# PeterFWS/Structure-PLP-SLAM

Measured on AMD Instinct MI355X. Metric: frames/sec ORB+LSD extract+match, 640x480 TUM-RGBD, 1/2/4/8 GPU, higher is better.
Workload: dtype u8

## Files before the change

structure-plp-slam_amd/csrc/line_context.hip:

```cpp
#include <hip/hip_runtime.h>

#include <algorithm>
#include <cmath>
#include <cstring>
#include <mutex>
#include <vector>

#include "line_device.hpp"
#include "null4.hpp"
#include "seed_sort_model.hpp"
#include "sincos_ziv.hpp"
#include "plp_common.hpp"

using namespace plp;

struct plp_line {
    HostPinned pin;
    int device = 0;
    hipStream_t stream = nullptr;
    hipStream_t idle_stream = nullptr;
    int rows = 0, cols = 0, capB = 0;
    int grow_waves = 0;
    int seed_order = PLP_SEED_ORDER_LIBSTDCXX;
    bool mw_ok = false, seed_sort_ok = false;
// ... 3 lines not shown
    ResizeExactTab rt{};
    BlurTapsN t11{}, t5{};
    LbdWeightsDev w{};
    DevBuf tabs, blur11, scaled, pix, g2, maxgrad, undef, order, n_order, reg, mw_heap, seed_ent, seed_ws, raw, n_raw, dx, dy, all_kl, all_kl_dir, all_lbd, n_all, status, prof, grow_stats;
    DevBuf l0copy, s_kl, s_lbd, s_fn, s_cnt;
    DevBuf aligned;
    int s_cap = 0;
    int last_B = 0;
    bool last_profiled = false;
    hipStream_t last_stream = nullptr;
    bool profiling = false;
    bool grow_big_ok = false;
    hipEvent_t ev[9] = {};
    double stage_ms[9] = {0, 0, 0, 0, 0, 0, 0, 0, 0};
    long stage_batches = 0;
    std::mutex mu;
};

namespace {

void gaussian_taps(int n, double sigma, int* out) {
    std::vector<double> k(n);
    double sum = 0;
    for (int i = 0; i < n; ++i) { const double x = i - (n - 1) * 0.5; k[i] = std::exp(-0.5 / (sigma * sigma) * x * x); sum += k[i]; }
    double err = 0;
    int acc = 0;
    for (int i = 0; i < n / 2; ++i) {
        const double adj = k[i] / sum * 256.0 + err;
        const int v = (int)std::nearbyint(adj);
        err = adj - v;
        out[i] = out[n - 1 - i] = v;
        acc += v;
    }
    out[n / 2] = 256 - 2 * acc;
}

int floor_d(double v) { int i = (int)v; return i - (i > v); }

void exact_coeffs(int ssize, int dsize, std::vector<int16_t>& ofs, std::vector<int16_t>& c1) {
    const double scale = 1.0 / ((double)dsize / ssize);
    for (int d = 0; d < dsize; ++d) {
        const double val = ((double)d + 0.5) * scale - 0.5;
        const int iv = floor_d(val);
        if (iv >= 0 && ssize > 1) {
            if (iv < ssize - 1) { ofs.push_back((int16_t)iv); c1.push_back((int16_t)std::nearbyint((val - (double)iv) * 256.0)); }
            else { ofs.push_back((int16_t)(ssize - 1)); c1.push_back(-1); }
        } else { ofs.push_back(0); c1.push_back(-2); }
    }
}

plp_status build(plp_line* c, int rows, int cols) {
    if (c->rows == rows && c->cols == cols) return PLP_OK;
    if (rows < 16 || cols < 16 || rows > 16000 || cols > 16000) return set_error(PLP_ERR_INVALID_ARG, "unsupported frame size for the line front-end");
    LinePlanes& P = c->P;
    P.W = cols; P.H = rows;
    P.sw = (int)std::nearbyint(cols * 0.5); P.sh = (int)std::nearbyint(rows * 0.5);
    P.sw_magic = (P.sw >= 2 && P.sw <= 8192) ? (uint32_t)(((1ull << 32) + (uint64_t)P.sw - 1) / (uint64_t)P.sw) : 0u;
    if (P.sw >= 65536 || P.sh >= 65536 || (size_t)P.sw * P.sh > kLsdMaxScaledPixels || (!c->grow_big_ok && (size_t)P.sw * P.sh > 516065))
        return set_error(PLP_ERR_UNSUPPORTED, "frame too large for the LSD region-growing kernel (the half-resolution image must not exceed 524,257 pixels: a 1920 x 1080 frame is the largest common one)");
    P.pitch = (cols + 63) / 64 * 64; P.spitch = (P.sw + 63) / 64 * 64;
    LsdParams& lp = c->lp;
    const double ang_th = 22.5, quant = 2.0;
    lp.prec = M_PI * ang_th / 180; lp.p = ang_th / 180; lp.rho = quant / std::sin(lp.prec);
    lp.c_pass = (float)std::cos(lp.prec - kLsdAngleBand); lp.c_fail = (float)std::cos(lp.prec + kLsdAngleBand);
    {
        uint32_t g = 0;
        while (g < 600000u && std::sqrt((double)g / 4.0) <= lp.rho) ++g;
        lp.g2_def_min = g;
    }
    lp.density_th = 0.6; lp.scale = 0.5; lp.n_bins = 1024; lp.refine = 1;
    const double LOG_NT = 5 * (std::log10((double)P.sw) + std::log10((double)P.sh)) / 2 + std::log10(11.0);
    lp.min_reg_size = (int)(size_t)(-LOG_NT / std::log10(lp.p));
    lp.min_length = (float)(0.125 * std::min(cols, rows));
    lp.keep_length = 60.f;
    const double sigma = 0.6 / 0.5;
    const unsigned h = (unsigned)std::ceil(sigma * std::sqrt(2 * 3.0 * std::log(10.0)));
    if (h != 5) return set_error(PLP_ERR_UNSUPPORTED, "unexpected LSD kernel size");
    gaussian_taps(11, sigma, c->t11.k);
    for (int i = 0; i < 11; ++i) c->t5.k[i] = 0;
    gaussian_taps(5, 1.0, c->t5.k);
    {
        double u = (7 * 3 - 1) / 2, sg = (7 * 2 + 1) / 2, inv = -1 / (2 * sg * sg);
        for (int i = 0; i < 21; ++i) { const double d = i - u; c->w.l[i] = (float)std::exp(d * d * inv); }
        u = (9 * 7 - 1) / 2; sg = u; inv = -1 / (2 * sg * sg);
        for (int i = 0; i < 63; ++i) { const double d = i - u; c->w.g[i] = (float)std::exp(d * d * inv); }
    }
    std::vector<int16_t> xo, xc, yo, yc;
    exact_coeffs(cols, P.sw, xo, xc);
    exact_coeffs(rows, P.sh, yo, yc);
    {
        bool plain = cols == 2 * P.sw && rows == 2 * P.sh;
        for (int i = 0; plain && i < P.sw; ++i) plain = xo[i] == 2 * i && xc[i] == 128;
        for (int i = 0; plain && i < P.sh; ++i) plain = yo[i] == 2 * i && yc[i] == 128;
        P.half_exact = plain ? 1 : 0;
    }
    std::vector<int16_t> blob;
    blob.insert(blob.end(), xo.begin(), xo.end()); blob.insert(blob.end(), xc.begin(), xc.end());
    blob.insert(blob.end(), yo.begin(), yo.end()); blob.insert(blob.end(), yc.begin(), yc.end());
    PLP_HIP(c->tabs.upload(blob.data(), blob.size() * 2, c->stream));
    PLP_HIP(hipStreamSynchronize(c->stream));
    const int16_t* base = (const int16_t*)c->tabs.p;
    c->rt.xo = base; c->rt.xc = base + P.sw; c->rt.yo = base + 2 * P.sw; c->rt.yc = base + 2 * P.sw + P.sh;
    c->rows = rows; c->cols = cols; c->capB = 0; c->mw_capB = 0; c->seed_capB = 0;
    return PLP_OK;
}

plp_status ensure(plp_line* c, int B) {
    LinePlanes& P = c->P;
    const size_t n = (size_t)P.sw * P.sh, nv = (size_t)(P.sw - 1) * (P.sh - 1);
    const int Bmw = std::min(B, kLsdMwMaxFrames);
    if (B > c->capB) {
        if (!P.half_exact) PLP_HIP(c->blur11.reserve((size_t)P.pitch * P.H * B));
        PLP_HIP(c->scaled.reserve((size_t)P.spitch * P.sh * B));
        PLP_HIP(c->pix.reserve(n * sizeof(LsdPix) * B));
        PLP_HIP(c->g2.reserve(n * 4 * B)); PLP_HIP(c->n_order.reserve(4 * (size_t)B)); PLP_HIP(c->maxgrad.reserve(4 * ((n + 255) / 256) * (size_t)B)); PLP_HIP(c->undef.reserve((n + 63) / 64 * 8 * B));
        PLP_HIP(c->order.reserve(nv * 4 * B)); PLP_HIP(c->reg.reserve(std::max(n * (size_t)B, 2 * n * (size_t)Bmw) * 4));
        PLP_HIP(c->raw.reserve(sizeof(float4) * kLineCap * B)); PLP_HIP(c->n_raw.reserve(4 * (size_t)B));
        PLP_HIP(c->dx.reserve(dxy_frame_entries(P.W, P.H) * 4 * B));
        PLP_HIP(c->all_kl.reserve(sizeof(plp_keyline) * kLineCap * B)); PLP_HIP(c->all_kl_dir.reserve(sizeof(float2) * kLineCap * B)); PLP_HIP(c->all_lbd.reserve((size_t)32 * kLineCap * B));
        PLP_HIP(c->n_all.reserve(4 * (size_t)B)); PLP_HIP(c->status.reserve(16)); PLP_HIP(c->prof.reserve(128)); PLP_HIP(c->grow_stats.reserve(16 * (size_t)B));
        P.blur11 = (uint8_t*)c->blur11.p; P.scaled = (uint8_t*)c->scaled.p;
        P.pix = (LsdPix*)c->pix.p; P.g2 = (uint32_t*)c->g2.p; P.n_order = (int32_t*)c->n_order.p;
        P.blockmax = (uint32_t*)c->maxgrad.p; P.undef = (unsigned long long*)c->undef.p;
        P.order = (uint32_t*)c->order.p; P.reg = (uint32_t*)c->reg.p; P.raw = (float4*)c->raw.p; P.n_raw = (int32_t*)c->n_raw.p;
        P.dxy = (short2*)c->dx.p; P.all_kl = (plp_keyline*)c->all_kl.p; P.all_kl_dir = (float2*)c->all_kl_dir.p; P.all_lbd = (uint8_t*)c->all_lbd.p;
        P.n_all = (int32_t*)c->n_all.p; P.status = (int32_t*)c->status.p; P.prof = (long long*)c->prof.p; P.grow_stats = (int32_t*)c->grow_stats.p;
        c->capB = B;
    }
    P.reg_frame_stride = B <= kLsdMwMaxFrames ? 2 * n : n;
    P.mw_heap_frame_stride = (size_t)(kMwMaxWaves - 1) * kMwHeapBufs * kMwHeap;
    if (c->mw_ok && B <= kLsdMwMaxFrames && B > c->mw_capB) {
        PLP_HIP(c->mw_heap.reserve(P.mw_heap_frame_stride * 4 * (size_t)B));
        c->mw_capB = B;
    }
    P.mw_heap = (B <= c->mw_capB) ? (uint32_t*)c->mw_heap.p : nullptr;
    if (c->seed_order == PLP_SEED_ORDER_LIBSTDCXX && B > c->seed_capB) {
        PLP_HIP(c->seed_ent.reserve(nv * 4 * (size_t)B)); PLP_HIP(c->seed_ws.reserve(seed_sort_ws_entries(nv) * 4 * (size_t)B));
        c->seed_capB = B;
    }
    return PLP_OK;
}

plp_status run(plp_line* c, const uint8_t* d_imgs, int B, int rows, int cols, size_t step, size_t frame_stride, plp_keyline* d_kl,
               uint8_t* d_lbd, double* d_fn, int cap, int32_t* d_counts, hipStream_t st) {
    PLP_HIP(hipSetDevice(c->device));
    if (c->seed_order == PLP_SEED_ORDER_LIBSTDCXX && !c->seed_sort_ok)
        return set_error(PLP_ERR_UNSUPPORTED, "this device refused the dynamic LDS size of the exact seed sort (144 KB per workgroup): select PLP_SEED_ORDER_STABLE with plp_line_set_seed_order");
    PLP_TRY(build(c, rows, cols));
    PLP_TRY(ensure(c, B));
    if (((uintptr_t)d_imgs % 4 == 0) && (step % 4 == 0) && (frame_stride % 4 == 0)) {
        c->P.img = d_imgs; c->P.img_frame_stride = frame_stride; c->P.img_pitch = (int)step;
    } else {
        const size_t fs = (size_t)c->P.pitch * rows;
        PLP_HIP(c->aligned.reserve(fs * B));
        for (int f = 0; f < B; ++f)
            PLP_HIP(hipMemcpy2DAsync((uint8_t*)c->aligned.p + f * fs, c->P.pitch, d_imgs + f * frame_stride, step, cols, rows, hipMemcpyDeviceToDevice, st));
        c->P.img = (const uint8_t*)c->aligned.p; c->P.img_frame_stride = fs; c->P.img_pitch = c->P.pitch;
    }
    PLP_HIP(hipMemsetAsync(c->status.p, 0, 16, st));
    if (c->profiling) PLP_HIP(hipMemsetAsync(c->prof.p, 0, 128, st));
    const bool exact = c->seed_order == PLP_SEED_ORDER_LIBSTDCXX;
    c->lp.seed_exact = exact ? 1 : 0;
    const SeedSortBufs ssb{(uint32_t*)c->seed_ent.p, (uint32_t*)c->seed_ws.p, seed_sort_ws_entries((size_t)(c->P.sw - 1) * (c->P.sh - 1))};
    launch_line_front(st, c->P, c->lp, c->rt, c->t11, c->t5, c->w, d_kl, d_lbd, d_fn, cap, d_counts, B, c->profiling ? c->ev : nullptr,
                      c->grow_waves, exact ? &ssb : nullptr, c->mw_ok);
    PLP_HIP(hipGetLastError());
    if (c->profiling) {
        PLP_HIP(hipEventSynchronize(c->ev[8]));
        for (int i = 0; i < 8; ++i) { float ms = 0; PLP_HIP(hipEventElapsedTime(&ms, c->ev[i], c->ev[i + 1])); c->stage_ms[i] += ms; }
        float tot = 0; PLP_HIP(hipEventElapsedTime(&tot, c->ev[0], c->ev[8])); c->stage_ms[8] += tot;
        ++c->stage_batches;
    }
    c->last_B = B; c->last_stream = st; c->last_profiled = c->profiling;
    return PLP_OK;
}

plp_status batch_status(const int32_t s[4], bool check_cap) {
    if (check_cap && (s[0] & 1)) return set_error(PLP_ERR_CAPACITY, "a frame produced more lines than `cap`; output truncated");
    if (s[0] & 4) return set_error(PLP_ERR_OVERFLOW, "more LSD segments than the per-frame capacity");
    if (s[0] & 16) return set_error(PLP_ERR_HIP, "region growing with several waves per frame timed out in a wait (protocol error, please report the frame)");
    if (s[0] & 32) {
        static thread_local char msg[320];
        snprintf(msg, sizeof msg, "the exact seed sort stopped short in frame %d of the batch (reason %d: 1 = a partition's swap count / cut failed its check [m = %d], 2-3, 6-8 = a list or stack of its LDS ran out of space, "
                 "4-5 = a wave waited beyond the limit): the seed order of this batch is not guaranteed; please report the frame", s[2], s[1], s[3]);
        return set_error(PLP_ERR_OVERFLOW, msg);
    }
    return PLP_OK;
}

}

extern "C" {

plp_status plp_line_create(int device, plp_line** out) {
    if (!out) return set_error(PLP_ERR_INVALID_ARG, "out is NULL");
    *out = nullptr;
    int n = 0;
    if (hipGetDeviceCount(&n) != hipSuccess || n == 0) return set_error(PLP_ERR_NO_DEVICE, "no HIP device visible: the line front-end has no CPU fallback");
    if (device < 0 || device >= n) return set_error(PLP_ERR_INVALID_ARG, "device index out of range");
    PLP_HIP(hipSetDevice(device));
    plp_line* c = new plp_line();
    c->device = device;
    c->mw_ok = grow_mw_configure() == hipSuccess;
    c->grow_big_ok = grow_configure() == hipSuccess;
    c->seed_sort_ok = seed_sort_configure() == hipSuccess;
    (void)hipGetLastError();
    if (hipStreamCreateWithFlags(&c->stream, hipStreamNonBlocking) != hipSuccess) { delete c; return set_error(PLP_ERR_HIP, "hipStreamCreate failed"); }
    if (hipStreamCreateWithFlags(&c->idle_stream, hipStreamNonBlocking) != hipSuccess) c->idle_stream = nullptr;
    *out = c;
// ... 255 lines not shown
```

structure-plp-slam_amd/csrc/line_device.hpp:

```cpp
#pragma once
#include <hip/hip_runtime.h>
#include <stdint.h>

#include "../../include/plp_front.h"

namespace plp {

constexpr int kMwHeap = 16384;
constexpr int kMwHeapBufs = 2;
constexpr int kMwMaxWaves = 8;
constexpr int kLsdMwMaxFrames = 256;
constexpr int kLineCap = 2048;
constexpr double kLsdNotDef = -1024.0;
constexpr int kLsdSeedPixBits = 20;
constexpr uint32_t kLsdSeedPixMask = (1u << kLsdSeedPixBits) - 1u;
constexpr size_t kLsdGrowLdsBytes = 66560;
constexpr size_t kLsdMaxScaledPixels = (kLsdGrowLdsBytes / 4 - 256) * 32 - 31;
static_assert(kLsdMaxScaledPixels <= (size_t)kLsdSeedPixMask + 1, "seed packing of k_lsd_order must hold every admitted pixel index");
static_assert(kLsdSeedPixBits + 10 <= 32, "10 bits of gradient bin above the pixel field");

struct alignas(16) LsdPix { float deg; uint32_t g2; float2 cs; };
__device__ __forceinline__ double pix_ang(const LsdPix& p) { return (double)p.deg * (3.14159265358979323846 / 180); }
__device__ __forceinline__ double pix_mod(const LsdPix& p) { return sqrt((double)p.g2 / 4.0); }

struct LinePlanes {
    int W, H;
    int sw, sh;
    uint32_t sw_magic;
    int pitch, spitch;
    const uint8_t* img; size_t img_frame_stride; int img_pitch;
    uint8_t* blur11;
    uint8_t* scaled;
    LsdPix* pix;
    uint32_t* g2;
    uint32_t* blockmax;
    unsigned long long* undef;
    uint32_t* order;
    int32_t* n_order;
    uint32_t* reg; size_t reg_frame_stride;
    uint32_t* mw_heap; size_t mw_heap_frame_stride;
    float4* raw; int32_t* n_raw;
    short2* dxy;
    plp_keyline* all_kl; uint8_t* all_lbd; int32_t* n_all;
    float2* all_kl_dir;
    int32_t* status;
    int half_exact;
    int32_t* grow_stats;
    long long* prof;
};

__host__ __device__ inline size_t dxy_frame_entries(int W, int H) { return (size_t)((W + 7) / 8) * ((H + 3) / 4) * 32; }
__host__ __device__ inline int dxy_index(int x, int y, int tiles_x) { return (((y >> 2) * tiles_x + (x >> 3)) << 5) + ((y & 3) << 3) + (x & 7); }

struct LsdParams {
    double prec, p, rho, density_th, scale;
    int n_bins, refine, min_reg_size;
    float min_length;
    float keep_length;
    float c_pass, c_fail;
    uint32_t g2_def_min;
    int seed_exact;
};
constexpr double kLsdAngleBand = 3.5e-4;
constexpr double kLsdBandMinPrec = 0.01, kLsdBandMaxPrec = 1.5;

struct ResizeExactTab { const int16_t *xo, *xc, *yo, *yc; };
struct BlurTapsN { int k[11]; };
struct LbdWeightsDev { float g[63], l[21]; };

struct SeedSortBufs { uint32_t* ent; uint32_t* ws; size_t ws_stride; };
size_t seed_sort_ws_entries(size_t nv);
hipError_t seed_sort_configure();
void launch_seed_order_exact(hipStream_t st, const LinePlanes& P, const LsdParams& lp, int B, uint32_t* ent, uint32_t* ws, size_t ws_stride);
void launch_seed_sort_debug(hipStream_t st, uint32_t* ent, int n, int depth, uint32_t skip_key, uint32_t* ws, int32_t* status, int* dbg, int variant, int copies = 1);
hipError_t grow_mw_configure();
hipError_t grow_configure();

void launch_line_front(hipStream_t st, const LinePlanes& P, const LsdParams& lp, const ResizeExactTab& rt, const BlurTapsN& t11,
                       const BlurTapsN& t5, const LbdWeightsDev& w, plp_keyline* out_kl, uint8_t* out_lbd, double* out_fn, int cap,
                       int32_t* out_counts, int B, hipEvent_t* ev, int grow_waves, const SeedSortBufs* seed_exact, bool mw_ok);

}
```

structure-plp-slam_amd/csrc/line_kernels.hip:

```cpp
#include <hip/hip_runtime.h>
#include <stdint.h>

#include <algorithm>
#include <cstdlib>

#include "blur_tile.hpp"
#include "plp_barrier.hpp"
#include "line_device.hpp"
#include "plp_common.hpp"
#include "sincos_ziv.hpp"
#include "xcd_map.hpp"

namespace plp {

struct TileDiv { uint32_t gx_magic, tiles_x_magic; };
static inline TileDiv tile_div(int tiles, int tiles_x, int B) { return TileDiv{plp_div_magic((uint32_t)tiles, (uint64_t)tiles * B), plp_div_magic((uint32_t)tiles_x, (uint64_t)tiles)}; }

__device__ __forceinline__ int reflect101_l(int p, int len) {
    if (len == 1) return 0;
    while (p < 0 || p >= len) p = p < 0 ? -p : 2 * (len - 1) - p;
    return p;
}

__device__ __forceinline__ float fast_atan2_deg_l(float y, float x) {
// ... 1288 lines not shown
                    e->pos = t; e->n1 = r.n1; e->n2 = r.n2; e->nfinal = r.nfinal; e->flags = (r.keep ? 1u : 0u) | (r.second ? 2u : 0u); e->off = (uint32_t)hoff;
                    e->na = r.na; e->line = r.line;
                }
                if (tot <= kMwInline) {
                    if (lane < acc_n) e->inl[lane] = heap_ld(g.reg + lane);
                    else if (lane < tot) e->inl[lane] = g.assumed[lane - acc_n];
                }
                __builtin_amdgcn_fence(__ATOMIC_RELEASE, PLP_MW_SCOPE_NAME);
                __builtin_amdgcn_wave_barrier();
                ++nent; hoff += (tot + 1) & ~1;
                if (lds_ld(&pend_hi[h]) < 0) lds_st(&pend_lo[h], g.my_pos);
                lds_st(&pend_hi[h], g.my_pos);
                lds_st(&buf_n[h * kMwBufs + kbuf], nent);
                mw_forget(g, g.reg, acc_n, 0);
            } else mw_forget(g, g.reg, acc_n, wv);
            __builtin_amdgcn_wave_barrier();
            {
                const int p = (int)mine;
                const int ow = tent_owner(g, p), owh = ow > kMwPending ? ow - kMwPending : ow;
                const bool skip = committed(p) || (ow != 0 && (ow == kMwMainId || owh == wv || cur_pos[min(owh, kMwMaxWaves) - 1] < grp * kMwGroup + lane));
                todo &= __ballot(!skip);
            }
            lds_st(&hstate[h], (grp << 8) | (t + 1));
        }
    }
    if (is_main) {
        if (lane == 0) {
            P.n_raw[b] = min(n_lines, kLineCap);
            int32_t* gs = P.grow_stats + (size_t)b * 4; gs[0] = n_self; gs[1] = n_spec_ok; gs[2] = n_spec_bad; gs[3] = W;
            if (P.prof && b == 0 && prof_on) {
                P.prof[0] = now() - c_begin; P.prof[1] = c_wait; P.prof[2] = c_self;
                P.prof[3] = (long long)hcount[0] | ((long long)hcount[1] << 32); P.prof[4] = n_self; P.prof[5] = (long long)n_spec_ok | ((long long)n_spec_bad << 32);
                P.prof[6] = c_commit; P.prof[7] = c_pub; P.prof[8] = c_grp; P.prof[9] = P.prof[10] = P.prof[11] = 0;
            }
        }
        lds_st(done, 1);
    }
}

__global__ __launch_bounds__(64) void k_keylines(LinePlanes P, LsdParams lp) {
    const int b = blockIdx.x, lane = threadIdx.x;
    const int n = P.n_raw[b];
    const float4* raw = P.raw + (size_t)b * kLineCap;
    plp_keyline* out = P.all_kl + (size_t)b * kLineCap;
    int run = 0;
    for (int base = 0; base < n; base += 64) {
        const int i = base + lane;
        bool keep = false;
        plp_keyline kl{};
        if (i < n) {
            float4 e = raw[i];
            const float fw = (float)P.W, fh = (float)P.H;
            if (e.x < 0) e.x = 0;
            if (e.x >= fw) e.x = fw - 1.0f;
            if (e.z < 0) e.z = 0;
            if (e.z >= fw) e.z = fw - 1.0f;
            if (e.y < 0) e.y = 0;
            if (e.y >= fh) e.y = fh - 1.0f;
            if (e.w < 0) e.w = 0;
            if (e.w >= fh) e.w = fh - 1.0f;
            const double ddx = (double)__fsub_rn(e.x, e.z), ddy = (double)__fsub_rn(e.y, e.w);
            const double length = (double)(float)sqrt(ddx * ddx + ddy * ddy);
            keep = length > (double)lp.min_length;
            kl.startPointX = e.x; kl.startPointY = e.y; kl.endPointX = e.z; kl.endPointY = e.w;
            kl.sPointInOctaveX = e.x; kl.sPointInOctaveY = e.y; kl.ePointInOctaveX = e.z; kl.ePointInOctaveY = e.w;
            kl.lineLength = (float)length;
            const int x1 = __float2int_rn(e.x), y1 = __float2int_rn(e.y), x2 = __float2int_rn(e.z), y2 = __float2int_rn(e.w);
            kl.numOfPixels = max(abs(x2 - x1), abs(y2 - y1)) + 1;
            kl.angle = (float)atan2((double)__fsub_rn(e.w, e.y), (double)__fsub_rn(e.z, e.x));
            kl.octave = 0;
            kl.size = __fmul_rn(__fsub_rn(e.z, e.x), __fsub_rn(e.w, e.y));
            kl.response = __fdiv_rn(kl.lineLength, (float)max(P.W, P.H));
            kl.pt_x = __fdiv_rn(__fadd_rn(e.z, e.x), 2.0f);
            kl.pt_y = __fdiv_rn(__fadd_rn(e.w, e.y), 2.0f);
        }
        const unsigned long long bal = __ballot(keep);
        if (keep) {
            kl.class_id = run + __popcll(bal & ((1ull << lane) - 1ull));
            out[kl.class_id] = kl;
            P.all_kl_dir[(size_t)b * kLineCap + kl.class_id] = make_float2((float)cos((double)kl.angle), (float)sin((double)kl.angle));
        }
        run += __popcll(bal);
    }
    if (lane == 0) P.n_all[b] = run;
}

constexpr int kSobelTW = 120, kSobelTH = 30;
static_assert(sizeof(BlurTileLds<2>::in) >= kBlurTH * (kBlurTW / 4) * 4, "the blurred tile must fit the input rows it replaces");
__global__ __launch_bounds__(256) __attribute__((amdgpu_waves_per_eu(8, 8))) void k_blur_sobel(const uint8_t* __restrict__ src, size_t src_fs, int src_pitch,
                                                                                            short2* __restrict__ dxy, int w, int h, BlurTapsN taps, TileDiv td) {
    __shared__ __attribute__((aligned(16))) BlurTileLds<2> Sb;
    uint32_t* const bt = reinterpret_cast<uint32_t*>(Sb.in);
    const int tiles_x = (w + kSobelTW - 1) / kSobelTW;
    unsigned t, f;
    xcd_frame_major(t, f, td.gx_magic);
    const int trow = (int)plp_div(t, (unsigned)tiles_x, td.tiles_x_magic);
    const int bx0 = ((int)t - trow * tiles_x) * kSobelTW - 4, by0 = trow * kSobelTH - 1;
    blur_tile_core<2>(Sb, src + (size_t)f * src_fs, src_pitch, w, h, bx0, by0, taps.k, [&](int r0, int c4, const uint32_t (&rows)[kBlurRS]) {
#pragma unroll
        for (int rr = 0; rr < kBlurRS; ++rr) bt[(r0 + rr) * (kBlurTW / 4) + c4 / 4] = rows[rr];
    });
    wg_barrier();
    short2* out_frame = dxy + (size_t)f * dxy_frame_entries(w, h);
    const int tiles8 = (w + 7) / 8;
    for (int i = threadIdx.x; i < (kSobelTW / 4) * (kSobelTH / 2); i += 256) {
        const int cgp = i % (kSobelTW / 4), rp = i / (kSobelTW / 4);
        const int x = bx0 + 4 + 4 * cgp, y = by0 + 1 + 2 * rp;
        if (x >= w || y >= h) continue;
        const int cd = 1 + cgp;
        int d[4][4], sm[4][4];
#pragma unroll
        for (int r = 0; r < 4; ++r) {
            const uint32_t* q = &bt[(2 * rp + r) * (kBlurTW / 4) + cd];
            const uint32_t A = q[-1], Bv = q[0], Cv = q[1];
            const int p[6] = {(int)(A >> 24), (int)(Bv & 255u), (int)((Bv >> 8) & 255u), (int)((Bv >> 16) & 255u), (int)(Bv >> 24), (int)(Cv & 255u)};
#pragma unroll
            for (int k = 0; k < 4; ++k) { d[r][k] = p[k + 2] - p[k]; sm[r][k] = p[k] + 2 * p[k + 1] + p[k + 2]; }
        }
#pragma unroll
        for (int j = 0; j < 2; ++j) {
            if (y + j >= h) continue;
            uint32_t out[4];
#pragma unroll
            for (int k = 0; k < 4; ++k)
                out[k] = ((uint32_t)(d[j][k] + 2 * d[j + 1][k] + d[j + 2][k]) & 0xffffu) | ((uint32_t)(sm[j + 2][k] - sm[j][k]) << 16);
            *reinterpret_cast<uint4*>(out_frame + dxy_index(x, y + j, tiles8)) = make_uint4(out[0], out[1], out[2], out[3]);
        }
    }
}

__constant__ int c_comb[32][2] = {{0, 1}, {0, 2}, {0, 3}, {0, 4}, {0, 5}, {0, 6}, {1, 2}, {1, 3}, {1, 4}, {1, 5}, {1, 6},
                                  {2, 3}, {2, 4}, {2, 5}, {2, 6}, {2, 7}, {2, 8}, {3, 4}, {3, 5}, {3, 6}, {3, 7}, {3, 8},
                                  {4, 5}, {4, 6}, {4, 7}, {4, 8}, {5, 6}, {5, 7}, {5, 8}, {6, 7}, {6, 8}, {7, 8}};

constexpr int kLbdU = 8;
__global__ __launch_bounds__(256) void k_lbd(LinePlanes P, LbdWeightsDev W) {
    __shared__ float s_row[4][63][8];
    __shared__ float s_des[4][72], s_des2[4][72], s_norm[4][4];
    const int lane = threadIdx.x & 63, wv = __builtin_amdgcn_readfirstlane((int)(threadIdx.x >> 6)), b = blockIdx.y;
    const int n_lines = P.n_all[b];
    for (int li = blockIdx.x * 4 + wv; li < n_lines; li += gridDim.x * 4) {
    const plp_keyline kl = P.all_kl[(size_t)b * kLineCap + li];
    const short2* dxyImg = P.dxy + (size_t)b * dxy_frame_entries(P.W, P.H);
    const int tiles8 = (P.W + 7) / 8;
    const short imageWidth = (short)(P.W - 1), imageHeight = (short)(P.H - 1);
    const short lengthOfLSP = (short)kl.numOfPixels;
    const short halfWidth = (short)((lengthOfLSP - 1) / 2), halfHeight = 31;
    const float midX = (float)(0.5 * (double)__fadd_rn(kl.sPointInOctaveX, kl.ePointInOctaveX));
    const float midY = (float)(0.5 * (double)__fadd_rn(kl.sPointInOctaveY, kl.ePointInOctaveY));
    const float2 dir = P.all_kl_dir[(size_t)b * kLineCap + li];
    const float dL0 = dir.x, dL1 = dir.y;
    const float dO0 = -dL1, dO1 = dL0;
    if (lane < 63) {
        float sCorX0 = __fadd_rn(__fadd_rn(__fmul_rn(-dL0, (float)halfWidth), __fmul_rn(dL1, (float)halfHeight)), midX);
        float sCorY0 = __fadd_rn(__fsub_rn(__fmul_rn(-dL1, (float)halfWidth), __fmul_rn(dL0, (float)halfHeight)), midY);
        for (int r = 0; r < lane; ++r) { sCorX0 = __fsub_rn(sCorX0, dL1); sCorY0 = __fadd_rn(sCorY0, dL0); }
        float sCorX = sCorX0, sCorY = sCorY0;
        float pgdL = 0, ngdL = 0, pgdO = 0, ngdO = 0;
        for (int w0 = 0; w0 < lengthOfLSP; w0 += kLbdU) {
            int off[kLbdU];
#pragma unroll
            for (int u = 0; u < kLbdU; ++u) {
                short t = (short)roundf(sCorX);
                const short xCor = (t < 0) ? 0 : (t > imageWidth) ? imageWidth : t;
                t = (short)roundf(sCorY);
                const short yCor = (t < 0) ? 0 : (t > imageHeight) ? imageHeight : t;
                off[u] = dxy_index(xCor, yCor, tiles8);
                sCorX = __fadd_rn(sCorX, dL0);
                sCorY = __fadd_rn(sCorY, dL1);
            }
            short2 vxy[kLbdU];
#pragma unroll
            for (int u = 0; u < kLbdU; ++u) vxy[u] = dxyImg[off[u]];
#pragma unroll
            for (int u = 0; u < kLbdU; ++u) {
                if (w0 + u < lengthOfLSP) {
                    const float fx = (float)vxy[u].x, fy = (float)vxy[u].y;
                    const float gDL = __fadd_rn(__fmul_rn(fx, dL0), __fmul_rn(fy, dL1));
                    const float gDO = __fadd_rn(__fmul_rn(fx, dO0), __fmul_rn(fy, dO1));
                    if (gDL > 0) pgdL = __fadd_rn(pgdL, gDL); else ngdL = __fsub_rn(ngdL, gDL);
                    if (gDO > 0) pgdO = __fadd_rn(pgdO, gDO); else ngdO = __fsub_rn(ngdO, gDO);
                }
            }
        }
        const float cg = W.g[lane];
        pgdL = __fmul_rn(cg, pgdL); ngdL = __fmul_rn(cg, ngdL); pgdO = __fmul_rn(cg, pgdO); ngdO = __fmul_rn(cg, ngdO);
        float* r = s_row[wv][lane];
        r[0] = pgdL; r[1] = ngdL; r[2] = __fmul_rn(pgdL, pgdL); r[3] = __fmul_rn(ngdL, ngdL);
        r[4] = pgdO; r[5] = ngdO; r[6] = __fmul_rn(pgdO, pgdO); r[7] = __fmul_rn(ngdO, ngdO);
    }
    __builtin_amdgcn_fence(__ATOMIC_RELEASE, "workgroup");
    __builtin_amdgcn_wave_barrier();
    for (int item = lane; item < 72; item += 64) {
        const int band = item >> 3, comp = item & 7;
        const bool sq = (comp == 2 || comp == 3 || comp == 6 || comp == 7);
        float acc = 0;
        for (int hID = max(0, (band - 1) * 7); hID < min(63, (band + 2) * 7); ++hID) {
            const int rb = hID / 7;
            const float c = rb == band ? W.l[hID % 7 + 7] : (rb == band + 1 ? W.l[hID % 7 + 14] : W.l[hID % 7]);
            const float v = s_row[wv][hID][comp];
            acc = sq ? __fadd_rn(acc, __fmul_rn(__fmul_rn(c, c), v)) : __fadd_rn(acc, __fmul_rn(c, v));
        }
        s_des[wv][item] = acc;
    }
    __builtin_amdgcn_fence(__ATOMIC_RELEASE, "workgroup");
    __builtin_amdgcn_wave_barrier();
    float* des = s_des2[wv];
    auto wave_sync = [] { __builtin_amdgcn_fence(__ATOMIC_ACQ_REL, "workgroup"); __builtin_amdgcn_wave_barrier(); };
    if (lane < 36) {
        const int band = lane >> 2, k = lane & 3;
        const float invN = (band == 0 || band == 8) ? (float)(1.0 / (7 * 2.0)) : (float)(1.0 / (7 * 3.0));
        const float* sb = &s_des[wv][band * 8];
        const int mi = (k < 2) ? k : k + 2, qi = mi + 2;
        const float temp = __fmul_rn(sb[mi], invN);
        des[band * 8 + k] = temp;
        des[band * 8 + 4 + k] = sqrtf(__fsub_rn(__fmul_rn(sb[qi], invN), __fmul_rn(temp, temp)));
    }
    wave_sync();
    if (lane == 0) {
        float tempM = 0, tempS = 0;
        for (int band = 0; band < 9; ++band) {
            const float* v = des + 8 * band;
            for (int k = 0; k < 4; ++k) tempM = __fadd_rn(tempM, __fmul_rn(v[k], v[k]));
            for (int k = 4; k < 8; ++k) tempS = __fadd_rn(tempS, __fmul_rn(v[k], v[k]));
        }
        s_norm[wv][0] = __fdiv_rn(1.0f, sqrtf(tempM));
        s_norm[wv][1] = __fdiv_rn(1.0f, sqrtf(tempS));
    }
    wave_sync();
    for (int i = lane; i < 72; i += 64) {
        float v = __fmul_rn(des[i], s_norm[wv][(i >> 2) & 1]);
        if ((double)v > 0.4) v = (float)0.4;
        des[i] = v;
    }
    wave_sync();
    if (lane == 0) {
        float temp = 0;
        for (int i = 0; i < 72; ++i) temp = __fadd_rn(temp, __fmul_rn(des[i], des[i]));
        s_norm[wv][2] = __fdiv_rn(1.0f, sqrtf(temp));
    }
    wave_sync();
    for (int i = lane; i < 72; i += 64) des[i] = __fmul_rn(des[i], s_norm[wv][2]);
    wave_sync();
    if (lane < 32) {
        const float* f1 = des + 8 * c_comb[lane][0];
        const float* f2 = des + 8 * c_comb[lane][1];
        unsigned r = 0;
        for (int i = 0; i < 8; ++i) r += (f1[i] > f2[i]) ? (1u << i) : 0u;
        P.all_lbd[((size_t)b * kLineCap + li) * 32 + lane] = (uint8_t)r;
    }
    __builtin_amdgcn_fence(__ATOMIC_ACQ_REL, "workgroup");
    __builtin_amdgcn_wave_barrier();
    }
}

__global__ __launch_bounds__(64) void k_line_finalize(LinePlanes P, LsdParams lp, plp_keyline* __restrict__ out_kl,
                                                      uint8_t* __restrict__ out_lbd, double* __restrict__ out_fn, int cap,
                                                      int32_t* __restrict__ out_counts) {
    const int b = blockIdx.x, lane = threadIdx.x;
    const int n = P.n_all[b];
    int run = 0;
    for (int base = 0; base < n; base += 64) {
        const int i = base + lane;
        plp_keyline kl{};
        bool keep = false;
        if (i < n) { kl = P.all_kl[(size_t)b * kLineCap + i]; keep = kl.octave == 0 && kl.lineLength >= lp.keep_length; }
        const unsigned long long bal = __ballot(keep);
        const int o = run + __popcll(bal & ((1ull << lane) - 1ull));
        if (keep && o < cap) {
            out_kl[(size_t)b * cap + o] = kl;
            const uint4* s = reinterpret_cast<const uint4*>(P.all_lbd + ((size_t)b * kLineCap + i) * 32);
            uint4* d = reinterpret_cast<uint4*>(out_lbd + ((size_t)b * cap + o) * 32);
            d[0] = s[0]; d[1] = s[1];
            const double sx = kl.startPointX, sy = kl.startPointY, ex = kl.endPointX, ey = kl.endPointY;
            const double a = sy * 1.0 - 1.0 * ey, bb = 1.0 * ex - sx * 1.0, c = sx * ey - sy * ex;
            const double nrm = sqrt(a * a + bb * bb);
            double* f = out_fn + ((size_t)b * cap + o) * 3;
            f[0] = a / nrm; f[1] = bb / nrm; f[2] = c / nrm;
        }
        run += __popcll(bal);
    }
    if (lane == 0) {
        out_counts[b] = min(run, cap);
        if (run > cap) atomicOr(P.status, 1);
    }
}

void launch_line_front(hipStream_t st, const LinePlanes& P, const LsdParams& lp, const ResizeExactTab& rt, const BlurTapsN& t11,
                       const BlurTapsN& t5, const LbdWeightsDev& w, plp_keyline* out_kl, uint8_t* out_lbd, double* out_fn, int cap,
                       int32_t* out_counts, int B, hipEvent_t* ev, int grow_waves, const SeedSortBufs* seed_exact, bool mw_ok) {
    auto mark = [&](int i) { if (ev) (void)hipEventRecord(ev[i], st); };
    const bool sobel_first = !ev;
    const size_t plane_fs = (size_t)P.pitch * P.H, splane_fs = (size_t)P.spitch * P.sh;
    const int tiles = ((P.W + 127) / 128) * ((P.H + kBlurTH - 1) / kBlurTH);
    const int sobel_tiles = ((P.W + kSobelTW - 1) / kSobelTW) * ((P.H + kSobelTH - 1) / kSobelTH);
    const TileDiv blur_td = tile_div(tiles, (P.W + 127) / 128, B), sobel_td = tile_div(sobel_tiles, (P.W + kSobelTW - 1) / kSobelTW, B);
    mark(0);
    if (sobel_first) hipLaunchKernelGGL(k_blur_sobel, dim3(sobel_tiles, B), dim3(256), 0, st, P.img, P.img_frame_stride, P.img_pitch, P.dxy, P.W, P.H, t5, sobel_td);
    if (P.half_exact)
        hipLaunchKernelGGL(k_blur_half, dim3(tiles, B), dim3(256), 0, st, P.img, P.img_frame_stride, P.img_pitch, P.scaled, splane_fs, P.spitch, P.W, P.H, t11, blur_td);
    else {
        hipLaunchKernelGGL(k_blur_plane<5>, dim3(tiles, B), dim3(256), 0, st, P.img, P.img_frame_stride, P.img_pitch, P.blur11, plane_fs,
                           P.pitch, P.W, P.H, t11, blur_td);
        hipLaunchKernelGGL(k_resize_exact, dim3((P.sw + 255) / 256, (P.sh + 3) / 4, B), dim3(64, 4), 0, st, P.blur11, plane_fs, P.pitch,
                           P.scaled, splane_fs, P.spitch, P.sw, P.sh, rt);
    }
    mark(1);
    const int n = P.sw * P.sh;
    hipLaunchKernelGGL(k_lsd_gradient, dim3((n + 255) / 256, B), dim3(256), 0, st, P, lp);
    mark(2);
    if (seed_exact) launch_seed_order_exact(st, P, lp, B, seed_exact->ent, seed_exact->ws, seed_exact->ws_stride);
    else hipLaunchKernelGGL(k_lsd_order, dim3(B), dim3(256), 0, st, P, lp, (n + 255) / 256);
    mark(3);
    constexpr int ring = 256;
    const size_t per_wave = (size_t)((((n + 31) / 32 + 1) & ~1) + ring) * 4;
    const int wpb = (int)std::max<size_t>(1, std::min<size_t>(4, 65536 / per_wave));
    MwLayout L{};
    size_t mw_bytes = 0;
    const int want_waves = grow_waves > 0 ? std::min(grow_waves, kMwMaxWaves) : kMwMaxWaves;
    if (mw_ok && B <= kLsdMwMaxFrames && want_waves >= 2 && P.mw_heap && P.reg_frame_stride >= 2 * (size_t)n) {
        const int nw_al = (((n + 31) / 32 + 1) & ~1), groups_cap = ((P.sw - 1) * (P.sh - 1) + kMwGroup - 1) / kMwGroup + 64 / kMwGroup;
        for (int w = want_waves; w >= 2; --w) {
            const size_t bytes = (size_t)5 * nw_al * 4 + (size_t)w * (nw_al + 256 + kMwAssumed + 2) * 4 + (8 + (4 + 2 * kMwBufs) * kMwMaxWaves) * 4 + ((groups_cap + 15) & ~15) + 16 +
                                 (size_t)(w - 1) * kMwBufs * kMwEntries * sizeof(MwEntry);
            if (bytes <= 160 * 1024) { L.waves = w; L.ring = 256; L.nw_al = nw_al; L.n_groups_cap = groups_cap; L.lookahead = kMwBufs * (w - 1); L.policy = 0; L.prof = ev ? 1 : 0; mw_bytes = bytes; break; }
        }
    }
    if (L.waves >= 2)
        hipLaunchKernelGGL(k_lsd_grow_mw, dim3(B), dim3(64 * L.waves), mw_bytes, st, P, lp, L);
    else
        hipLaunchKernelGGL(k_lsd_grow, dim3((B + wpb - 1) / wpb), dim3(64 * wpb), per_wave * wpb, st, P, lp, B, wpb, ring);
    mark(4);
    hipLaunchKernelGGL(k_keylines, dim3(B), dim3(64), 0, st, P, lp);
    mark(5);
    if (!sobel_first) hipLaunchKernelGGL(k_blur_sobel, dim3(sobel_tiles, B), dim3(256), 0, st, P.img, P.img_frame_stride, P.img_pitch, P.dxy, P.W, P.H, t5, sobel_td);
    mark(6);
    const int lbd_blocks = B >= 64 ? 2 : 16;
    hipLaunchKernelGGL(k_lbd, dim3(lbd_blocks, B), dim3(256), 0, st, P, w);
    mark(7);
    hipLaunchKernelGGL(k_line_finalize, dim3(B), dim3(64), 0, st, P, lp, out_kl, out_lbd, out_fn, cap, out_counts);
    mark(8);
}

hipError_t grow_configure() {
    return hipFuncSetAttribute(reinterpret_cast<const void*>(k_lsd_grow), hipFuncAttributeMaxDynamicSharedMemorySize, (int)kLsdGrowLdsBytes);
}
hipError_t grow_mw_configure() {
    return hipFuncSetAttribute(reinterpret_cast<const void*>(k_lsd_grow_mw), hipFuncAttributeMaxDynamicSharedMemorySize, (int)(160 * 1024));
}

}
```

Before: 95300.

## Rework LBD descriptor kernel with atomic line tickets and inside-image fast path

The LBD kernel now hands out lines to waves through a per-frame atomic ticket counter (reset in k_keylines) instead of a static stride, which balances uneven line lengths. A bounding-box test lets fully interior lines skip clamping and use simpler rounding and offset math. The band accumulation is restructured with zero-padded rows and precomputed squared coefficients in LDS, and the norm reductions read precomputed squares with vector loads. The grid for large batches also grows from 2 to 3 blocks per frame. Risks include floating-point ordering differences and the atomic's overhead.

After: 96850 (median of 6 runs). 1.6% higher.

```diff
diff --git a/structure-plp-slam_amd/csrc/line_context.hip b/structure-plp-slam_amd/csrc/line_context.hip
--- a/structure-plp-slam_amd/csrc/line_context.hip
+++ b/structure-plp-slam_amd/csrc/line_context.hip
@@ -109,6 +109,7 @@
     {
         double u = (7 * 3 - 1) / 2, sg = (7 * 2 + 1) / 2, inv = -1 / (2 * sg * sg);
         for (int i = 0; i < 21; ++i) { const double d = i - u; c->w.l[i] = (float)std::exp(d * d * inv); }
+        for (int i = 0; i < 21; ++i) c->w.l2[i] = c->w.l[i] * c->w.l[i];
         u = (9 * 7 - 1) / 2; sg = u; inv = -1 / (2 * sg * sg);
         for (int i = 0; i < 63; ++i) { const double d = i - u; c->w.g[i] = (float)std::exp(d * d * inv); }
     }
@@ -145,13 +146,13 @@
         PLP_HIP(c->raw.reserve(sizeof(float4) * kLineCap * B)); PLP_HIP(c->n_raw.reserve(4 * (size_t)B));
         PLP_HIP(c->dx.reserve(dxy_frame_entries(P.W, P.H) * 4 * B));
         PLP_HIP(c->all_kl.reserve(sizeof(plp_keyline) * kLineCap * B)); PLP_HIP(c->all_kl_dir.reserve(sizeof(float2) * kLineCap * B)); PLP_HIP(c->all_lbd.reserve((size_t)32 * kLineCap * B));
-        PLP_HIP(c->n_all.reserve(4 * (size_t)B)); PLP_HIP(c->status.reserve(16)); PLP_HIP(c->prof.reserve(128)); PLP_HIP(c->grow_stats.reserve(16 * (size_t)B));
+        PLP_HIP(c->n_all.reserve(8 * (size_t)B));    PLP_HIP(c->status.reserve(16)); PLP_HIP(c->prof.reserve(128)); PLP_HIP(c->grow_stats.reserve(16 * (size_t)B));
         P.blur11 = (uint8_t*)c->blur11.p; P.scaled = (uint8_t*)c->scaled.p;
         P.pix = (LsdPix*)c->pix.p; P.g2 = (uint32_t*)c->g2.p; P.n_order = (int32_t*)c->n_order.p;
         P.blockmax = (uint32_t*)c->maxgrad.p; P.undef = (unsigned long long*)c->undef.p;
         P.order = (uint32_t*)c->order.p; P.reg = (uint32_t*)c->reg.p; P.raw = (float4*)c->raw.p; P.n_raw = (int32_t*)c->n_raw.p;
         P.dxy = (short2*)c->dx.p; P.all_kl = (plp_keyline*)c->all_kl.p; P.all_kl_dir = (float2*)c->all_kl_dir.p; P.all_lbd = (uint8_t*)c->all_lbd.p;
-        P.n_all = (int32_t*)c->n_all.p; P.status = (int32_t*)c->status.p; P.prof = (long long*)c->prof.p; P.grow_stats = (int32_t*)c->grow_stats.p;
+        P.n_all = (int32_t*)c->n_all.p; P.lbd_ticket = P.n_all + B; P.status = (int32_t*)c->status.p; P.prof = (long long*)c->prof.p; P.grow_stats = (int32_t*)c->grow_stats.p;
         c->capB = B;
     }
     P.reg_frame_stride = B <= kLsdMwMaxFrames ? 2 * n : n;
diff --git a/structure-plp-slam_amd/csrc/line_device.hpp b/structure-plp-slam_amd/csrc/line_device.hpp
--- a/structure-plp-slam_amd/csrc/line_device.hpp
+++ b/structure-plp-slam_amd/csrc/line_device.hpp
@@ -43,6 +43,7 @@
     short2* dxy;
     plp_keyline* all_kl; uint8_t* all_lbd; int32_t* n_all;
     float2* all_kl_dir;
+    int32_t* lbd_ticket;
     int32_t* status;
     int half_exact;
     int32_t* grow_stats;
@@ -66,7 +67,7 @@
 
 struct ResizeExactTab { const int16_t *xo, *xc, *yo, *yc; };
 struct BlurTapsN { int k[11]; };
-struct LbdWeightsDev { float g[63], l[21]; };
+struct LbdWeightsDev { float g[63], l[21], l2[21]; };
 
 struct SeedSortBufs { uint32_t* ent; uint32_t* ws; size_t ws_stride; };
 size_t seed_sort_ws_entries(size_t nv);
diff --git a/structure-plp-slam_amd/csrc/line_kernels.hip b/structure-plp-slam_amd/csrc/line_kernels.hip
--- a/structure-plp-slam_amd/csrc/line_kernels.hip
+++ b/structure-plp-slam_amd/csrc/line_kernels.hip
@@ -1394,7 +1394,7 @@
         }
         run += __popcll(bal);
     }
-    if (lane == 0) P.n_all[b] = run;
+    if (lane == 0) { P.n_all[b] = run; P.lbd_ticket[b] = 0; }
 }
 
 constexpr int kSobelTW = 120, kSobelTH = 30;
@@ -1446,120 +1446,190 @@
                                   {4, 5}, {4, 6}, {4, 7}, {4, 8}, {5, 6}, {5, 7}, {5, 8}, {6, 7}, {6, 8}, {7, 8}};
 
 constexpr int kLbdU = 8;
+
+__device__ __forceinline__ void lbd_accumulate(uint32_t v, float dL0, float dL1, float& pgdL, float& ngdL, float& pgdO, float& ngdO) {
+    const float fx = (float)(short)(v & 0xffffu), fy = (float)(short)(v >> 16);
+    const float gDL = __fadd_rn(__fmul_rn(fx, dL0), __fmul_rn(fy, dL1));
+    const float gDO = __fadd_rn(__fmul_rn(fx, -dL1), __fmul_rn(fy, dL0));
+    pgdL = __fadd_rn(pgdL, fmaxf(gDL, 0.0f)); ngdL = __fsub_rn(ngdL, fminf(gDL, 0.0f));
+    pgdO = __fadd_rn(pgdO, fmaxf(gDO, 0.0f)); ngdO = __fsub_rn(ngdO, fminf(gDO, 0.0f));
+}
+
+template <bool kInside>
+__device__ __forceinline__ uint32_t lbd_sample_offset(float sx, float sy, short imageWidth, short imageHeight, uint32_t tile_row_bytes) {
+    uint32_t x, y;
+    if (kInside) {
+        x = (uint32_t)(int)__fadd_rn(sx, 0.5f);
+        y = (uint32_t)(int)__fadd_rn(sy, 0.5f);
+    } else {
+        short t = (short)roundf(sx);
+        x = (uint32_t)((t < 0) ? 0 : (t > imageWidth) ? imageWidth : t);
+        t = (short)roundf(sy);
+        y = (uint32_t)((t < 0) ? 0 : (t > imageHeight) ? imageHeight : t);
+    }
+    return __umul24(x & ~7u, 12u) + (x << 2) + __umul24(y >> 2, tile_row_bytes - 128u) + (y << 5);
+}
+
+template <bool kInside, bool kTail>
+__device__ __forceinline__ void lbd_trip(const char* __restrict__ dxyBytes, float& sCorX, float& sCorY, float dL0, float dL1, short imageWidth,
+                                         short imageHeight, uint32_t tile_row_bytes, int n, float& pgdL, float& ngdL, float& pgdO, float& ngdO) {
+    static_assert(!(kInside && kTail), "the steps past a line's end may leave the image: the tail trip clamps");
+    uint32_t off[kLbdU];
+#pragma unroll
+    for (int u = 0; u < kLbdU; ++u) {
+        off[u] = lbd_sample_offset<kInside>(sCorX, sCorY, imageWidth, imageHeight, tile_row_bytes);
+        sCorX = __fadd_rn(sCorX, dL0);
+        sCorY = __fadd_rn(sCorY, dL1);
+    }
+    uint32_t vxy[kLbdU];
+#pragma unroll
+    for (int u = 0; u < kLbdU; ++u) vxy[u] = *reinterpret_cast<const uint32_t*>(dxyBytes + off[u]);
+#pragma unroll
+    for (int u = 0; u < kLbdU; ++u)
+        if (!kTail || u < n) lbd_accumulate(vxy[u], dL0, dL1, pgdL, ngdL, pgdO, ngdO);
+}
+
+constexpr int kLbdPad = 7;
 __global__ __launch_bounds__(256) void k_lbd(LinePlanes P, LbdWeightsDev W) {
-    __shared__ float s_row[4][63][8];
-    __shared__ float s_des[4][72], s_des2[4][72], s_norm[4][4];
+    __shared__ float s_row[4][63 + 2 * kLbdPad][8];
+    __shared__ __attribute__((aligned(16))) float s_des[4][72], s_des2[4][72], s_sq[4][72];
+    __shared__ float s_norm[4][4];
+    __shared__ float s_coef[2][21];
     const int lane = threadIdx.x & 63, wv = __builtin_amdgcn_readfirstlane((int)(threadIdx.x >> 6)), b = blockIdx.y;
     const int n_lines = P.n_all[b];
-    for (int li = blockIdx.x * 4 + wv; li < n_lines; li += gridDim.x * 4) {
+    const char* dxyBytes = reinterpret_cast<const char*>(P.dxy + (size_t)b * dxy_frame_entries(P.W, P.H));
+    const uint32_t tile_row_bytes = (uint32_t)((P.W + 7) / 8) * 128u;
+    const short imageWidth = (short)(P.W - 1), imageHeight = (short)(P.H - 1);
+    auto wave_sync = [] { __builtin_amdgcn_fence(__ATOMIC_ACQ_REL, "workgroup"); __builtin_amdgcn_wave_barrier(); };
+    if (lane < 2 * kLbdPad) {
+        float* z = s_row[wv][lane < kLbdPad ? lane : 63 + lane];
+#pragma unroll
+        for (int k = 0; k < 8; ++k) z[k] = 0.0f;
+    }
+    if (threadIdx.x < 21) { s_coef[0][threadIdx.x] = W.l[threadIdx.x]; s_coef[1][threadIdx.x] = W.l2[threadIdx.x]; }
+    wg_barrier();
+    for (;;) {
+    int li = 0;
+    if (lane == 0) li = atomicAdd(&P.lbd_ticket[b], 1);
+    li = __builtin_amdgcn_readfirstlane(li);
+    if (li >= n_lines) break;
     const plp_keyline kl = P.all_kl[(size_t)b * kLineCap + li];
-    const short2* dxyImg = P.dxy + (size_t)b * dxy_frame_entries(P.W, P.H);
-    const int tiles8 = (P.W + 7) / 8;
-    const short imageWidth = (short)(P.W - 1), imageHeight = (short)(P.H - 1);
     const short lengthOfLSP = (short)kl.numOfPixels;
     const short halfWidth = (short)((lengthOfLSP - 1) / 2), halfHeight = 31;
     const float midX = (float)(0.5 * (double)__fadd_rn(kl.sPointInOctaveX, kl.ePointInOctaveX));
     const float midY = (float)(0.5 * (double)__fadd_rn(kl.sPointInOctaveY, kl.ePointInOctaveY));
     const float2 dir = P.all_kl_dir[(size_t)b * kLineCap + li];
     const float dL0 = dir.x, dL1 = dir.y;
-    const float dO0 = -dL1, dO1 = dL0;
+    const float cornerX = __fadd_rn(__fadd_rn(__fmul_rn(-dL0, (float)halfWidth), __fmul_rn(dL1, (float)halfHeight)), midX);
+    const float cornerY = __fadd_rn(__fsub_rn(__fmul_rn(-dL1, (float)halfWidth), __fmul_rn(dL0, (float)halfHeight)), midY);
+    bool inside;
+    {
+        const float drift = (float)(62 + lengthOfLSP) * (float)(P.W + P.H) * 0x1p-22f;
+        const float ex = (float)(lengthOfLSP - 1) * dL0, ey = (float)(lengthOfLSP - 1) * dL1, rx = -62.0f * dL1, ry = 62.0f * dL0;
+        const float x_lo = cornerX + fminf(ex, 0.0f) + fminf(rx, 0.0f), x_hi = cornerX + fmaxf(ex, 0.0f) + fmaxf(rx, 0.0f);
+        const float y_lo = cornerY + fminf(ey, 0.0f) + fminf(ry, 0.0f), y_hi = cornerY + fmaxf(ey, 0.0f) + fmaxf(ry, 0.0f);
+        const bool in = x_lo >= 1.0f + drift && y_lo >= 1.0f + drift && x_hi <= (float)(P.W - 2) - drift && y_hi <= (float)(P.H - 2) - drift;
+        inside = __builtin_amdgcn_readfirstlane((int)in) != 0;
+    }
     if (lane < 63) {
-        float sCorX0 = __fadd_rn(__fadd_rn(__fmul_rn(-dL0, (float)halfWidth), __fmul_rn(dL1, (float)halfHeight)), midX);
-        float sCorY0 = __fadd_rn(__fsub_rn(__fmul_rn(-dL1, (float)halfWidth), __fmul_rn(dL0, (float)halfHeight)), midY);
-        for (int r = 0; r < lane; ++r) { sCorX0 = __fsub_rn(sCorX0, dL1); sCorY0 = __fadd_rn(sCorY0, dL0); }
-        float sCorX = sCorX0, sCorY = sCorY0;
+        float sCorX = cornerX, sCorY = cornerY;
+        for (int r = 0; r < lane; ++r) { sCorX = __fsub_rn(sCorX, dL1); sCorY = __fadd_rn(sCorY, dL0); }
         float pgdL = 0, ngdL = 0, pgdO = 0, ngdO = 0;
-        for (int w0 = 0; w0 < lengthOfLSP; w0 += kLbdU) {
-            int off[kLbdU];
-#pragma unroll
-            for (int u = 0; u < kLbdU; ++u) {
-                short t = (short)roundf(sCorX);
-                const short xCor = (t < 0) ? 0 : (t > imageWidth) ? imageWidth : t;
-                t = (short)roundf(sCorY);
-                const short yCor = (t < 0) ? 0 : (t > imageHeight) ? imageHeight : t;
-                off[u] = dxy_index(xCor, yCor, tiles8);
-                sCorX = __fadd_rn(sCorX, dL0);
-                sCorY = __fadd_rn(sCorY, dL1);
-            }
-            short2 vxy[kLbdU];
-#pragma unroll
-            for (int u = 0; u < kLbdU; ++u) vxy[u] = dxyImg[off[u]];
-#pragma unroll
-            for (int u = 0; u < kLbdU; ++u) {
-                if (w0 + u < lengthOfLSP) {
-                    const float fx = (float)vxy[u].x, fy = (float)vxy[u].y;
-                    const float gDL = __fadd_rn(__fmul_rn(fx, dL0), __fmul_rn(fy, dL1));
-                    const float gDO = __fadd_rn(__fmul_rn(fx, dO0), __fmul_rn(fy, dO1));
-                    if (gDL > 0) pgdL = __fadd_rn(pgdL, gDL); else ngdL = __fsub_rn(ngdL, gDL);
-                    if (gDO > 0) pgdO = __fadd_rn(pgdO, gDO); else ngdO = __fsub_rn(ngdO, gDO);
-                }
-            }
-        }
+        int w0 = 0;
+        if (inside)
+            for (; w0 + kLbdU <= lengthOfLSP; w0 += kLbdU)
+                lbd_trip<true, false>(dxyBytes, sCorX, sCorY, dL0, dL1, imageWidth, imageHeight, tile_row_bytes, kLbdU, pgdL, ngdL, pgdO, ngdO);
+        else
+            for (; w0 + kLbdU <= lengthOfLSP; w0 += kLbdU)
+                lbd_trip<false, false>(dxyBytes, sCorX, sCorY, dL0, dL1, imageWidth, imageHeight, tile_row_bytes, kLbdU, pgdL, ngdL, pgdO, ngdO);
+        if (w0 < lengthOfLSP)
+            lbd_trip<false, true>(dxyBytes, sCorX, sCorY, dL0, dL1, imageWidth, imageHeight, tile_row_bytes, lengthOfLSP - w0, pgdL, ngdL, pgdO, ngdO);
         const float cg = W.g[lane];
         pgdL = __fmul_rn(cg, pgdL); ngdL = __fmul_rn(cg, ngdL); pgdO = __fmul_rn(cg, pgdO); ngdO = __fmul_rn(cg, ngdO);
-        float* r = s_row[wv][lane];
+        float* r = s_row[wv][kLbdPad + lane];
         r[0] = pgdL; r[1] = ngdL; r[2] = __fmul_rn(pgdL, pgdL); r[3] = __fmul_rn(ngdL, ngdL);
         r[4] = pgdO; r[5] = ngdO; r[6] = __fmul_rn(pgdO, pgdO); r[7] = __fmul_rn(ngdO, ngdO);
     }
     __builtin_amdgcn_fence(__ATOMIC_RELEASE, "workgroup");
     __builtin_amdgcn_wave_barrier();
-    for (int item = lane; item < 72; item += 64) {
-        const int band = item >> 3, comp = item & 7;
-        const bool sq = (comp == 2 || comp == 3 || comp == 6 || comp == 7);
-        float acc = 0;
-        for (int hID = max(0, (band - 1) * 7); hID < min(63, (band + 2) * 7); ++hID) {
-            const int rb = hID / 7;
-            const float c = rb == band ? W.l[hID % 7 + 7] : (rb == band + 1 ? W.l[hID % 7 + 14] : W.l[hID % 7]);
-            const float v = s_row[wv][hID][comp];
-            acc = sq ? __fadd_rn(acc, __fmul_rn(__fmul_rn(c, c), v)) : __fadd_rn(acc, __fmul_rn(c, v));
-        }
-        s_des[wv][item] = acc;
+    int el = lane;
+    asm volatile("" : "+v"(el));
+    {
+        const int band = el >> 3, comp = el & 7;
+        const float* cf = s_coef[(comp >> 1) & 1];
+        const float* ra = &s_row[wv][band * 7][comp];
+        const float* rb = &s_row[wv][8 * 7][comp];
+        float acc = 0, acc8 = 0;
+#pragma unroll 1
+        for (int j0 = 0; j0 < 21; j0 += 7) {
+#pragma unroll
+            for (int j = 0; j < 7; ++j) {
+                const float c = cf[j0 + j];
+                acc = __fadd_rn(acc, __fmul_rn(c, ra[(j0 + j) * 8]));
+                acc8 = __fadd_rn(acc8, __fmul_rn(c, rb[(j0 + j) * 8]));
+            }
+        }
+        s_des[wv][el] = acc;
+        if (el < 8) s_des[wv][64 + el] = acc8;
     }
     __builtin_amdgcn_fence(__ATOMIC_RELEASE, "workgroup");
     __builtin_amdgcn_wave_barrier();
     float* des = s_des2[wv];
-    auto wave_sync = [] { __builtin_amdgcn_fence(__ATOMIC_ACQ_REL, "workgroup"); __builtin_amdgcn_wave_barrier(); };
-    if (lane < 36) {
-        const int band = lane >> 2, k = lane & 3;
+    float* dsq = s_sq[wv];
+    if (el < 36) {
+        const int band = el >> 2, k = el & 3;
         const float invN = (band == 0 || band == 8) ? (float)(1.0 / (7 * 2.0)) : (float)(1.0 / (7 * 3.0));
         const float* sb = &s_des[wv][band * 8];
         const int mi = (k < 2) ? k : k + 2, qi = mi + 2;
         const float temp = __fmul_rn(sb[mi], invN);
+        const float dev = sqrtf(__fsub_rn(__fmul_rn(sb[qi], invN), __fmul_rn(temp, temp)));
         des[band * 8 + k] = temp;
-        des[band * 8 + 4 + k] = sqrtf(__fsub_rn(__fmul_rn(sb[qi], invN), __fmul_rn(temp, temp)));
+        des[band * 8 + 4 + k] = dev;
+        dsq[band * 8 + k] = __fmul_rn(temp, temp);
+        dsq[band * 8 + 4 + k] = __fmul_rn(dev, dev);
     }
     wave_sync();
-    if (lane == 0) {
-        float tempM = 0, tempS = 0;
-        for (int band = 0; band < 9; ++band) {
-            const float* v = des + 8 * band;
-            for (int k = 0; k < 4; ++k) tempM = __fadd_rn(tempM, __fmul_rn(v[k], v[k]));
-            for (int k = 4; k < 8; ++k) tempS = __fadd_rn(tempS, __fmul_rn(v[k], v[k]));
-        }
-        s_norm[wv][0] = __fdiv_rn(1.0f, sqrtf(tempM));
-        s_norm[wv][1] = __fdiv_rn(1.0f, sqrtf(tempS));
+    if (el < 2) {
+        float acc = 0;
+#pragma unroll 1
+        for (int b0 = 0; b0 < 9; b0 += 3) {
+            float4 t[3];
+#pragma unroll
+            for (int q = 0; q < 3; ++q) t[q] = *reinterpret_cast<const float4*>(dsq + 8 * (b0 + q) + 4 * el);
+#pragma unroll
+            for (int q = 0; q < 3; ++q) acc = __fadd_rn(__fadd_rn(__fadd_rn(__fadd_rn(acc, t[q].x), t[q].y), t[q].z), t[q].w);
+        }
+        s_norm[wv][el] = __fdiv_rn(1.0f, sqrtf(acc));
     }
     wave_sync();
-    for (int i = lane; i < 72; i += 64) {
+    for (int i = el; i < 72; i += 64) {
         float v = __fmul_rn(des[i], s_norm[wv][(i >> 2) & 1]);
         if ((double)v > 0.4) v = (float)0.4;
         des[i] = v;
+        dsq[i] = __fmul_rn(v, v);
     }
     wave_sync();
-    if (lane == 0) {
+    if (el == 0) {
         float temp = 0;
-        for (int i = 0; i < 72; ++i) temp = __fadd_rn(temp, __fmul_rn(des[i], des[i]));
+#pragma unroll 1
+        for (int i0 = 0; i0 < 72; i0 += 24) {
+            float4 t[6];
+#pragma unroll
+            for (int q = 0; q < 6; ++q) t[q] = *reinterpret_cast<const float4*>(dsq + i0 + 4 * q);
+#pragma unroll
+            for (int q = 0; q < 6; ++q) temp = __fadd_rn(__fadd_rn(__fadd_rn(__fadd_rn(temp, t[q].x), t[q].y), t[q].z), t[q].w);
+        }
         s_norm[wv][2] = __fdiv_rn(1.0f, sqrtf(temp));
     }
     wave_sync();
-    for (int i = lane; i < 72; i += 64) des[i] = __fmul_rn(des[i], s_norm[wv][2]);
+    for (int i = el; i < 72; i += 64) des[i] = __fmul_rn(des[i], s_norm[wv][2]);
     wave_sync();
-    if (lane < 32) {
-        const float* f1 = des + 8 * c_comb[lane][0];
-        const float* f2 = des + 8 * c_comb[lane][1];
+    if (el < 32) {
+        const float* f1 = des + 8 * c_comb[el][0];
+        const float* f2 = des + 8 * c_comb[el][1];
         unsigned r = 0;
         for (int i = 0; i < 8; ++i) r += (f1[i] > f2[i]) ? (1u << i) : 0u;
-        P.all_lbd[((size_t)b * kLineCap + li) * 32 + lane] = (uint8_t)r;
+        P.all_lbd[((size_t)b * kLineCap + li) * 32 + el] = (uint8_t)r;
     }
     __builtin_amdgcn_fence(__ATOMIC_ACQ_REL, "workgroup");
     __builtin_amdgcn_wave_barrier();
@@ -1647,7 +1717,7 @@
     mark(5);
     if (!sobel_first) hipLaunchKernelGGL(k_blur_sobel, dim3(sobel_tiles, B), dim3(256), 0, st, P.img, P.img_frame_stride, P.img_pitch, P.dxy, P.W, P.H, t5, sobel_td);
     mark(6);
-    const int lbd_blocks = B >= 64 ? 2 : 16;
+    const int lbd_blocks = B >= 64 ? 3 : 16;
     hipLaunchKernelGGL(k_lbd, dim3(lbd_blocks, B), dim3(256), 0, st, P, w);
     mark(7);
     hipLaunchKernelGGL(k_line_finalize, dim3(B), dim3(64), 0, st, P, lp, out_kl, out_lbd, out_fn, cap, out_counts);
```
